# f78bono/deep-cine-cardiac-mri

Hardware: AMD Instinct MI355X
Metric: cine slices/sec, XF-VarNet R=4 15-coil 200x200x15t (higher is better)
Workload: dtype f32; 1 GPU; BASELINE.json configs[1]: XF-VarNet, 6 cascades, 15 coils x 15 frames x 200x200, R=4 Gaussian-density Cartesian mask, sens net 8ch/3 pools, U-Net 16ch/3 pools; 1 slice(s) per step (k-space batch axis), seeded random-init weights, 9 different slices per rank; parallelism=slice-sharded x1, one all-gather for volume assembly

## Files before the change

deep-cine-cardiac-mri_amd/cine_hip/dc.py:

```python
from typing import Optional

import torch

from . import autograd as ag
from . import ops


class Acquisition:
    def __init__(self, ref_kspace: torch.Tensor, mask: torch.Tensor, sens_maps: torch.Tensor, train: bool = False):
        layout = ops.mask_layout(mask, ref_kspace)
        if layout is None:
            raise ValueError(f"mask {tuple(mask.shape)} is in neither layout for k-space {tuple(ref_kspace.shape)}: pass it through ops.as_mask_u8")
        self.kspace, self.mask, self.sens, self.train = ref_kspace, mask, sens_maps, train
        self.row = layout == "row"
        self.fused = ops.general_mask_fused_train(mask, ref_kspace) if train else (self.row or ops.GENERAL_MASK_FUSED)
        self._hyb = self._zf = self._tiled = self._mf = None

    @property
    def tiled(self) -> Optional[torch.Tensor]:
        if self._tiled is None and self.row and not self.train:
            self._tiled = ops.sens_tile_pack(self.sens)
        return self._tiled

    @property
# ... 8 lines not shown
        self._hyb = ops.kspace_to_hybrid(self.kspace)
        return ops.hybrid_reduce(self._hyb, self.sens)

    def zero_filled(self) -> torch.Tensor:
        if self._zf is None:
            hyb, self._hyb = self._hyb, None
            if self.train:
                self._zf = ag.CoilReduceFn.apply(self.kspace, self.sens, self.mask)
            elif self.row:
                self._zf = ops.hybrid_reduce(ops.kspace_to_hybrid(self.kspace, out=hyb, mask=self.mask), self.sens)
            else:
                del hyb
                self._zf = ops.sens_reduce(ops.apply_mask(self.kspace, self.mask), self.sens, destroy_input=True)
        return self._zf

    def soft_dc(self, img: torch.Tensor, lambda_reg: torch.Tensor, magnitude: bool = False) -> torch.Tensor:
        if self.train:
            if self.row or self.fused:
                return ag.ImageDcFn.apply(img, self.sens, self.zero_filled(), self.mask, lambda_reg)
            k = ops.soft_dc_blend(ag.SensExpandFn.apply(img, self.sens, None), self.kspace, self.mask, lambda_reg)
            return ag.SensReduceFn.apply(k.contiguous(), self.sens, None)
        if self.fused:
            return ops.image_dc(img, self.sens, self.zero_filled(), self.mask, lambda_reg, magnitude=magnitude, sens_tiled=self.tiled)
        k = ops.soft_dc_blend(ops.sens_expand_dc(img, self.sens), self.kspace, self.mask, lambda_reg.detach())
        return ops.sens_reduce(k, self.sens, magnitude=magnitude, destroy_input=True)

    def residual_backward(self, x0: torch.Tensor) -> torch.Tensor:
        if self.train:
            if self.row or self.fused:
                return ag.ImageDcFixedFn.apply(x0, self.sens, self.zero_filled(), self.mask, 1.0, 0.0, -1.0)
            return ag.masked_residual_backward(x0, self.sens, self.kspace, self.mask)
        if self.fused:
            return ops.image_dc(x0, self.sens, self.zero_filled(), self.mask, weights=(1.0, 0.0, -1.0), sens_tiled=self.tiled)
        return ops.masked_residual_backward(x0, self.sens, self.kspace, self.mask)

    def forward_masked(self, x0: torch.Tensor) -> torch.Tensor:
        if self.train:
# ... 27 lines not shown
```

deep-cine-cardiac-mri_amd/cine_hip/ops.py:

```python
from typing import NamedTuple, Optional, Sequence

import contextlib
import ctypes
import threading
import numpy as np
import torch

from ._lib import CineHipError, check, lib

IN_EPS = 1e-5
LRELU_SLOPE = 0.2
RELU_ON = True
_act_tls = threading.local()


def lrelu_slope() -> float:
    return getattr(_act_tls, "slope", LRELU_SLOPE)


def relu_on() -> bool:
    return getattr(_act_tls, "relu", RELU_ON)


@contextlib.contextmanager
# ... 1211 lines not shown
    stats = torch.empty((n, 2, 2), device=x.device, dtype=x.dtype) if norm else None
    check(lib().cine_normunet_pack(x.data_ptr(), planes.data_ptr(), _p(stats), n, h, w, int(norm), _stream()),
          "cine_normunet_pack")
    return planes, stats


def normunet_unpack(planes: torch.Tensor, stats: Optional[torch.Tensor], h: int, w: int) -> torch.Tensor:
    planes = _dev(planes, "planes")
    n = planes.shape[0]
    y = torch.empty((n, h, w, 2), device=planes.device, dtype=planes.dtype)
    check(lib().cine_normunet_unpack(planes.data_ptr(), _p(stats), y.data_ptr(), n, h, w, _stream()),
          "cine_normunet_unpack")
    return y


def xfyf_pack(img: torch.Tensor, xf: bool, norm: bool = True):
    _pair(img)
    img = _dev(img, "image")
    b, t, h, w, _ = img.shape
    dev, dt = img.device, img.dtype
    pd = pad16 if norm else (lambda v: v)
    if pd(w) == pd(h):
        joint = torch.empty((b * h + b * w, 2, pd(w), pd(t)), device=dev, dtype=dt)
        pxf, pyf = joint[:b * h], joint[b * h:]
    else:
        pxf = torch.empty((b * h, 2, pd(w), pd(t)), device=dev, dtype=dt)
        pyf = torch.empty((b * w, 2, pd(h), pd(t)), device=dev, dtype=dt)
    sxf = torch.empty((b * h, 2, 2), device=dev, dtype=dt) if norm else None
    syf = torch.empty((b * w, 2, 2), device=dev, dtype=dt) if norm else None
    mean = torch.empty((b, h, w, 2), device=dev, dtype=dt)
    nbytes = lib().cine_xfyf_ws_bytes(b, t, h, w)
    ws = torch.empty(nbytes, device=dev, dtype=torch.uint8)
    check(lib().cine_xfyf_pack(img.data_ptr(), pxf.data_ptr(), pyf.data_ptr(), _p(sxf), _p(syf),
                               mean.data_ptr(), b, t, h, w, int(xf), int(norm), ws.data_ptr(), nbytes, _stream()),
          "cine_xfyf_pack")
    return pxf, pyf, sxf, syf, mean


def xfyf_unpack(pxf, pyf, sxf, syf, mean, b: int, t: int, h: int, w: int, xf: bool) -> torch.Tensor:
    out = torch.empty((b, t, 1, h, w, 2), device=pxf.device, dtype=pxf.dtype)
    check(lib().cine_xfyf_unpack(_dev(pxf, "pxf").data_ptr(), _dev(pyf, "pyf").data_ptr(), _p(sxf),
                                 _p(syf), mean.data_ptr(), out.data_ptr(), b, t, h, w, int(xf), _stream()),
          "cine_xfyf_unpack")
    return out


class _Kind(NamedTuple):
    stem: str
    dims: tuple
    tail: Optional[tuple]
    op: Optional[int]

    @property
    def floats_fn(self) -> str:
        return f"cine_{self.stem}_packed_floats"

    @property
    def pack_fn(self) -> str:
        return f"cine_pack_{self.stem}"
# ... 607 lines not shown
```

deep-cine-cardiac-mri_amd/csrc/fft_kernels.hip:

```cpp
#include <algorithm>
#include <map>
#include <mutex>
#include <utility>
#include "common.h"
#include "fft_core.h"

namespace cine {

__device__ const float2 TW200[200] = {
#include "tw200.inc"
};

constexpr int kLines200 = 32, kThreads200 = 320;
constexpr int kLinesGen = 8, kThreadsGen = 256;
constexpr int kMaxGenericN = 400;
constexpr int kMaxSmoothN = 512;
constexpr int kMaxOut = 4;

enum { POST_NONE = 0, POST_DC = 1, POST_HARD = 2, POST_RESID = 3, POST_W2D = 4,
       POST_LOSS = 5, POST_LOSSG = 6 };
constexpr bool post_plane(int post) { return post == POST_W2D || post == POST_LOSS || post == POST_LOSSG; }
constexpr bool post_kref(int post) { return post == POST_DC || post == POST_RESID || post == POST_LOSS || post == POST_LOSSG; }
enum { PRE_NONE = 0, PRE_SMUL = 1 };
enum { RPOST_NONE = 0, RPOST_REDUCE = 1, RPOST_REDUCE_ABS = 2, RPOST_RSS = 3,
// ... 1149 lines not shown
        ca.H = h; ca.W = w; ca.s_in = (h + 1) / 2; ca.s_out = h / 2; ca.coils = c;
        ca.premask = mask + (i0 / c) * h;
        if (int e = launch_col<POST_NONE, false, true>(ca, ni, true, st)) return e;
    }
    return CINE_OK;
}

extern "C" size_t cine_image_dc_ws_bytes(int b, int t, int c, int h, int w) {
    if (b <= 0 || t <= 0 || c <= 0 || h != 200 || w <= 0 || c <= kDcCS) return 0;
    return (size_t)ceil_div(c, kDcCS) * b * t * h * w * sizeof(cf);
}

static int image_dc_impl(const float* img, const float* sens, const float* zf, const uint8_t* mask,
                         const float* lambda_dev, int lam_beta, float w_sampled, float w_unsampled, float beta,
                         float* out, int b, int t, int c, int h, int w, int magnitude,
                         void* ws, size_t ws_bytes, void* stream, float* pd_part = nullptr, float* pd_wg = nullptr, const float* sens_tiled = nullptr);

extern "C" int cine_image_dc(const float* img, const float* sens, const float* zf, const uint8_t* mask,
                             const float* lambda_dev, float w_sampled, float w_unsampled, float beta,
                             float* out, int b, int t, int c, int h, int w, int magnitude,
                             void* ws, size_t ws_bytes, void* stream) {
    return image_dc_impl(img, sens, zf, mask, lambda_dev, 0, w_sampled, w_unsampled, beta, out, b, t, c, h, w, magnitude, ws, ws_bytes, stream);
}

extern "C" int cine_normal_op(const float* img, const float* sens, const uint8_t* mask, const float* lambda_dev,
                              float* out, int b, int t, int c, int h, int w, void* ws, size_t ws_bytes, void* stream) {
    CINE_REQUIRE(lambda_dev, CINE_EINVAL, "cine_normal_op: null lambda");
    return image_dc_impl(img, sens, img, mask, lambda_dev, 1, 1.f, 0.f, 0.f, out, b, t, c, h, w, 0, ws, ws_bytes, stream);
}
extern "C" size_t cine_sens_tile_floats(int b, int c, int h, int w) {
    return (b <= 0 || c <= 0 || h != 200 || w <= 0) ? 0 : (size_t)b * c * ceil_div(w, kDcCW) * 200 * kDcCW * 2;
// ... 16 lines not shown
    CINE_REQUIRE(sens && tiled, CINE_EINVAL, "cine_sens_tile_pack: null pointer");
    CINE_REQUIRE(b > 0 && c > 0 && h == 200 && w > 0, CINE_EUNSUPPORTED, "cine_sens_tile_pack: h must be 200 (the only engine that reads the tiled maps)");
    hipStream_t st = as_stream(stream);
    ProfScope prof(F_PACK, st);
    const long total = (long)b * c * ceil_div(w, kDcCW) * 200 * kDcCW;
    hipLaunchKernelGGL(sens_tile_pack_kernel, dim3((unsigned)std::min<long>(ceil_div(total, 256L), 4096)), dim3(256), 0, st,
                       reinterpret_cast<const cf*>(sens), reinterpret_cast<cf*>(tiled), w, ceil_div(w, kDcCW), (long)b * c);
    return check_launch("sens_tile_pack_kernel");
}
extern "C" int cine_image_dc_t(const float* img, const float* sens, const float* sens_tiled, const float* zf, const uint8_t* mask,
                               const float* lambda_dev, float w_sampled, float w_unsampled, float beta,
                               float* out, int b, int t, int c, int h, int w, int magnitude,
                               void* ws, size_t ws_bytes, void* stream) {
    return image_dc_impl(img, sens, zf, mask, lambda_dev, 0, w_sampled, w_unsampled, beta, out, b, t, c, h, w, magnitude, ws, ws_bytes, stream,
                         nullptr, nullptr, sens_tiled);
}
extern "C" int cine_normal_op_t(const float* img, const float* sens, const float* sens_tiled, const uint8_t* mask, const float* lambda_dev,
                                float* out, int b, int t, int c, int h, int w, void* ws, size_t ws_bytes, void* stream) {
    CINE_REQUIRE(lambda_dev, CINE_EINVAL, "cine_normal_op_t: null lambda");
    return image_dc_impl(img, sens, img, mask, lambda_dev, 1, 1.f, 0.f, 0.f, out, b, t, c, h, w, 0, ws, ws_bytes, stream, nullptr, nullptr, sens_tiled);
}
extern "C" int cine_normal_op_pd(const float* img, const float* sens, const uint8_t* mask, const float* lambda_dev,
                                 float* out, float* pd_part, int b, int t, int c, int h, int w, void* ws, size_t ws_bytes, void* stream) {
    CINE_REQUIRE(lambda_dev && pd_part, CINE_EINVAL, "cine_normal_op_pd: null pointer");
    CINE_REQUIRE(cine_image_dc_ws_bytes(b, t, c, h, w) > 0, CINE_EUNSUPPORTED, "cine_normal_op_pd: this shape has no partial-sum kernel");
    return image_dc_impl(img, sens, img, mask, lambda_dev, 1, 1.f, 0.f, 0.f, out, b, t, c, h, w, 0, ws, ws_bytes, stream, pd_part);
}

namespace cine {
int launch_cg_update_fused(float* x, float* r, float* p, const cf* partial, int nz, long part_stride, const float* lam, long ncf,
// ... 93 lines not shown
        a.cg_p_out = pk;
        {
            ProfScope prof(F_FFT_COL, st);
            hipLaunchKernelGGL(imgdc200_kernel<true>, dim3((unsigned)nb), dim3(kDcT), (size_t)200 * kDcL * sizeof(cf), st, a);
            if (int e = check_launch("imgdc200_kernel<cg>")) return e;
        }
        if (int e = launch_cg_update2(x, pr, pk, partial, nz, ncf, lambda_dev, ncf, pd_wg, (int)nb, rr[k & 1], rr[(k + 1) & 1], k + 1 == iters, st,
                                      rr_rec ? rr_rec + k : nullptr, pd_rec ? pd_rec + k : nullptr, (rr_rec && k + 1 == iters) ? rr_rec + iters : nullptr)) return e;
    }
    return CINE_OK;
}

static int image_dc_impl(const float* img, const float* sens, const float* zf, const uint8_t* mask,
                         const float* lambda_dev, int lam_beta, float w_sampled, float w_unsampled, float beta,
                         float* out, int b, int t, int c, int h, int w, int magnitude,
                         void* ws, size_t ws_bytes, void* stream, float* pd_part, float* pd_wg, const float* sens_tiled) {
    CINE_REQUIRE(img && sens && mask && (out || pd_wg), CINE_EINVAL, "cine_image_dc: null pointer");
    CINE_REQUIRE(b > 0 && t > 0 && c > 0 && h > 0 && w > 0, CINE_EINVAL, "cine_image_dc: bad sizes");
    CINE_REQUIRE((long)b * t <= 65535, CINE_EUNSUPPORTED, "cine_image_dc: b*t > 65535");
    CINE_REQUIRE(img != out, CINE_EINVAL, "cine_image_dc: out must not alias img (workgroups read neighbouring columns' rows)");
    if (int e = check_n(h, "cine_image_dc(h)")) return e;
    const size_t need = cine_image_dc_ws_bytes(b, t, c, h, w);
    CINE_REQUIRE(need == 0 || (ws && ws_bytes >= need), CINE_EWORKSPACE, "cine_image_dc: workspace %zu < %zu", ws_bytes, need);
    ImgDcArgs a{};
    a.img = reinterpret_cast<const cf*>(img); a.sens = reinterpret_cast<const cf*>(sens);
    a.zf = reinterpret_cast<const cf*>(zf); a.mask = mask; a.lam = lambda_dev; a.lam_beta = lam_beta;
    a.w1 = w_sampled; a.w0 = w_unsampled; a.beta = beta;
    a.out = magnitude ? nullptr : reinterpret_cast<cf*>(out); a.out_abs = magnitude ? out : nullptr;
    a.T = t; a.C = c; a.H = h; a.W = w;
    hipStream_t st = as_stream(stream);
    ProfScope prof(F_FFT_COL, st);
    if (h == 200) {
        const int nz = ceil_div(c, kDcCS);
        CINE_REQUIRE(nz <= 65535, CINE_EUNSUPPORTED, "cine_image_dc: %d coils", c);
        a.partial = reinterpret_cast<cf*>(ws); a.part_stride = (long)b * t * h * w;
        a.BT = b * t; a.ntx = ceil_div(w, kDcCW); a.nz = nz;
        a.sens_t = reinterpret_cast<const cf*>(sens_tiled);
        const long nblk = 8L * ceil_div(a.ntx * nz, 8) * a.BT;
        CINE_REQUIRE(nblk <= 0x7fffffffL, CINE_EUNSUPPORTED, "cine_image_dc: grid too large");
        CINE_REQUIRE(!pd_wg || nz > 1, CINE_EUNSUPPORTED, "cine_image_dc: per-workgroup dot partials need more than one coil group");
        a.pd_wg = pd_wg;
        hipLaunchKernelGGL(imgdc200_kernel<false>, dim3((unsigned)nblk), dim3(kDcT), (size_t)200 * kDcL * sizeof(cf), st, a);
        if (int e = check_launch("imgdc200_kernel")) return e;
        if (nz > 1 && !pd_wg) {
            const long n = a.part_stride;
            a.pd_part = pd_part;
            hipLaunchKernelGGL(imgdc_sum_kernel, dim3(pd_part ? 256u : (unsigned)std::min<long>(ceil_div(n, 256L), 2048)), dim3(256), 0, st, a, nz, n);
        }
    } else {
        const size_t lds = lds_bytes(false, h, kLinesGen);
        if (int e = allow_lds(imgdc_generic_kernel, lds, "imgdc_generic_kernel")) return e;
        hipLaunchKernelGGL(imgdc_generic_kernel, dim3(ceil_div(w, kLinesGen), b * t), dim3(kThreadsGen), lds, st, a);
    }
    return check_launch("imgdc_kernel");
}

extern "C" int cine_hybrid_reduce(const float* hyb, const float* sens, float* out,
                                  int b, int t, int c, int h, int w, int magnitude, void* stream) {
    CINE_REQUIRE(hyb && sens && out, CINE_EINVAL, "cine_hybrid_reduce: null pointer");
// ... 341 lines not shown
```

deep-cine-cardiac-mri_amd/csrc/pack_kernels.hip:

```cpp
#include <algorithm>
#include "common.h"
#include "fft_core.h"

namespace cine {

__device__ __forceinline__ float wave_sum(float v) {
#pragma unroll
    for (int o = 32; o > 0; o >>= 1) v += __shfl_xor(v, o, 64);
    return v;
}
__device__ __forceinline__ float block_sum(float v, float* red) {
    v = wave_sum(v);
    const int wave = threadIdx.x >> 6, nw = (blockDim.x + 63) >> 6;
    __syncthreads();
    if ((threadIdx.x & 63) == 0) red[wave] = v;
    __syncthreads();
    float s = 0.f;
    for (int i = 0; i < nw; ++i) s += red[i];
    return s;
}

struct PackArgs {
    const float* x; float* planes; float* stats;
    int n, I, J, Ip, Jp, pad_i, pad_j;
// ... 114 lines not shown
    if (stats) { const float* st = stats + (long)n * 4; mr = st[0]; sdr = st[1]; mi = st[2]; sdi = st[3]; }
    const float* pr = planes + (long)n * 2 * Ip * Jp;
    const float* pi = pr + (long)Ip * Jp;
    for (int e = blockIdx.x * blockDim.x + threadIdx.x; e < I * J; e += gridDim.x * blockDim.x) {
        const int i = e / J, j = e - i * J;
        const int q = (i + pad_i) * Jp + (j + pad_j);
        float2 v;
        v.x = pr[q] * sdr + mr;
        v.y = pi[q] * sdi + mi;
        reinterpret_cast<float2*>(y)[(long)n * I * J + e] = v;
    }
}

constexpr int kPix = 64;

__device__ __forceinline__ void temporal_table(cf* tw, int T) {
    const double s = 1.0 / sqrt((double)T);
    for (int j = threadIdx.x; j < T; j += blockDim.x) {
        double sn, cs;
        sincospi(2.0 * (double)j / (double)T, &sn, &cs);
        tw[j] = mk((float)(cs * s), (float)(-sn * s));
    }
}

__global__ void temporal_fwd_kernel(const cf* img, cf* X, cf* mean_img, int T, long HW, int xf) {
    extern __shared__ __align__(16) unsigned char smem[];
    cf* buf = reinterpret_cast<cf*>(smem);
    cf* tw = buf + T * kPix;
    const int b = blockIdx.y;
    const long p0 = (long)blockIdx.x * kPix;
    const int np = (int)min((long)kPix, HW - p0);
    if (xf) temporal_table(tw, T);
    for (int e = threadIdx.x; e < T * kPix; e += blockDim.x) {
        const int t = e / kPix, p = e - t * kPix;
        buf[e] = p < np ? img[((long)b * T + t) * HW + p0 + p] : mk(0.f, 0.f);
    }
    __syncthreads();
    if (threadIdx.x < kPix) {
        const int p = threadIdx.x;
        float sx = 0.f, sy = 0.f;
        for (int t = 0; t < T; ++t) { sx += buf[t * kPix + p].x; sy += buf[t * kPix + p].y; }
        const cf m = mk(sx / T, sy / T);
        for (int t = 0; t < T; ++t) buf[t * kPix + p] = csub(buf[t * kPix + p], m);
        if (p < np) mean_img[(long)b * HW + p0 + p] = m;
    }
    __syncthreads();
    const int s_in = (T + 1) / 2, s_out = T / 2;
    for (int e = threadIdx.x; e < np * T; e += blockDim.x) {
        const int p = e / T, i = e - p * T;
        cf r;
// ... 7 lines not shown
                ax += x.x * w.x - x.y * w.y; ay += x.x * w.y + x.y * w.x;
                idx += k; if (idx >= T) idx -= T;
            }
            r = mk(ax, ay);
        } else {
            r = buf[i * kPix + p];
        }
        X[((long)b * HW + p0 + p) * T + i] = r;
    }
}

struct UnpackArgs {
    const float* pxf; const float* pyf; const float* sxf; const float* syf;
    const cf* mean_img; cf* out;
    int T, H, W, Tp, Hp, Wp, pad_t, pad_h, pad_w, xf;
};

__global__ void xfyf_unpack_kernel(UnpackArgs a) {
    extern __shared__ __align__(16) unsigned char smem[];
    cf* buf = reinterpret_cast<cf*>(smem);
    cf* tw = buf + a.T * kPix;
    const int T = a.T, H = a.H, W = a.W;
    const int b = blockIdx.z, h = blockIdx.y;
    const int w0 = blockIdx.x * kPix;
    const int np = min(kPix, W - w0);
    if (a.xf) temporal_table(tw, T);
    const long nxf = (long)b * H + h;
    float xmr = 0.f, xsr = 1.f, xmi = 0.f, xsi = 1.f;
    if (a.sxf) { const float* sx = a.sxf + nxf * 4; xmr = sx[0]; xsr = sx[1]; xmi = sx[2]; xsi = sx[3]; }
    const float* pxr = a.pxf + nxf * 2 * a.Wp * a.Tp;
    const float* pxi = pxr + (long)a.Wp * a.Tp;
    for (int e = threadIdx.x; e < np * T; e += blockDim.x) {
        const int p = e / T, t = e - p * T;
        const int w = w0 + p;
        const int qx = (w + a.pad_w) * a.Tp + t + a.pad_t;
        const float xr = pxr[qx] * xsr + xmr, xi = pxi[qx] * xsi + xmi;
        const long nyf = (long)b * W + w;
        float ymr = 0.f, ysr = 1.f, ymi = 0.f, ysi = 1.f;
        if (a.syf) { const float* sy = a.syf + nyf * 4; ymr = sy[0]; ysr = sy[1]; ymi = sy[2]; ysi = sy[3]; }
        const float* pyr = a.pyf + nyf * 2 * a.Hp * a.Tp;
        const float* pyi = pyr + (long)a.Hp * a.Tp;
// ... 102 lines not shown
extern "C" int cine_normunet_unpack(const float* planes, const float* stats, float* y, int n, int h, int w, void* stream) {
    CINE_REQUIRE(planes && y, CINE_EINVAL, "cine_normunet_unpack: null pointer");
    CINE_REQUIRE(n > 0 && n <= 65535 && h > 0 && w > 0, CINE_EINVAL, "cine_normunet_unpack: bad sizes");
    int hp, ph, wp, pw;
    pad_split(h, hp, ph, stats != nullptr); pad_split(w, wp, pw, stats != nullptr);
    ProfScope prof(F_PACK, as_stream(stream));
    hipLaunchKernelGGL(normunet_unpack_kernel, dim3(grid_for((long)h * w, 256, 64), n), dim3(256), 0, as_stream(stream),
                       planes, stats, y, h, w, hp, wp, ph, pw);
    return check_launch("normunet_unpack_kernel");
}

extern "C" size_t cine_xfyf_ws_bytes(int b, int t, int h, int w) {
    return (size_t)b * t * h * w * 2 * sizeof(float);
}

extern "C" int cine_xfyf_pack(const float* img, float* planes_xf, float* planes_yf, float* stats_xf, float* stats_yf,
                              float* mean_img, int b, int t, int h, int w, int xf, int norm, void* ws, size_t ws_bytes, void* stream) {
    CINE_REQUIRE(img && planes_xf && planes_yf && mean_img && ws && (!norm || (stats_xf && stats_yf)), CINE_EINVAL,
                 "cine_xfyf_pack: null pointer");
    CINE_REQUIRE(b > 0 && b <= 65535 && t > 1 && h > 0 && w > 0, CINE_EINVAL, "cine_xfyf_pack: bad sizes");
    CINE_REQUIRE(t <= 64, CINE_EUNSUPPORTED, "cine_xfyf_pack: %d frames > 64", t);
    CINE_REQUIRE(ws_bytes >= cine_xfyf_ws_bytes(b, t, h, w), CINE_EWORKSPACE, "cine_xfyf_pack: workspace too small");
    hipStream_t st = as_stream(stream);
    cf* X = reinterpret_cast<cf*>(ws);
    const long HW = (long)h * w;
    const size_t lds = ((size_t)t * kPix + t) * sizeof(cf);
    ProfScope prof(F_PACK, st);
    hipLaunchKernelGGL(temporal_fwd_kernel, dim3((unsigned)ceil_div(HW, (long)kPix), b), dim3(256), lds, st,
                       reinterpret_cast<const cf*>(img), X, reinterpret_cast<cf*>(mean_img), t, HW, xf);
    if (int e = check_launch("temporal_fwd_kernel")) return e;
    PackArgs a{};
    a.x = reinterpret_cast<const float*>(X); a.planes = planes_xf; a.stats = stats_xf;
    a.n = b * h; a.I = w; a.J = t; a.norm = norm != 0;
    pad_split(w, a.Ip, a.pad_i, a.norm); pad_split(t, a.Jp, a.pad_j, a.norm);
    a.ninner = h; a.s_outer = HW * t * 2; a.s_inner = (long)w * t * 2; a.si = (long)t * 2; a.sj = 2;
    const PackArgs axf = a;
    a.planes = planes_yf; a.stats = stats_yf;
    a.n = b * w; a.I = h; a.J = t;
    pad_split(h, a.Ip, a.pad_i, a.norm); pad_split(t, a.Jp, a.pad_j, a.norm);
    a.ninner = w; a.s_outer = HW * t * 2; a.s_inner = (long)t * 2; a.si = (long)w * t * 2; a.sj = 2;
    return launch_pack(axf, &a, st);
}

extern "C" int cine_xfyf_unpack(const float* planes_xf, const float* planes_yf, const float* stats_xf,
                                const float* stats_yf, const float* mean_img, float* out,
                                int b, int t, int h, int w, int xf, void* stream) {
    CINE_REQUIRE(planes_xf && planes_yf && mean_img && out && ((stats_xf != nullptr) == (stats_yf != nullptr)), CINE_EINVAL,
                 "cine_xfyf_unpack: null pointer");
    CINE_REQUIRE(b > 0 && t > 1 && t <= 64 && h > 0 && w > 0 && h <= 65535 && b <= 65535, CINE_EINVAL,
                 "cine_xfyf_unpack: bad sizes");
    UnpackArgs a{};
    a.pxf = planes_xf; a.pyf = planes_yf; a.sxf = stats_xf; a.syf = stats_yf;
    a.mean_img = reinterpret_cast<const cf*>(mean_img); a.out = reinterpret_cast<cf*>(out);
    a.T = t; a.H = h; a.W = w; a.xf = xf;
    const bool nrm = stats_xf != nullptr;
    pad_split(t, a.Tp, a.pad_t, nrm); pad_split(h, a.Hp, a.pad_h, nrm); pad_split(w, a.Wp, a.pad_w, nrm);
    const size_t lds = ((size_t)t * kPix + t) * sizeof(cf);
    ProfScope prof(F_PACK, as_stream(stream));
    hipLaunchKernelGGL(xfyf_unpack_kernel, dim3(ceil_div(w, kPix), h, b), dim3(256), lds, as_stream(stream), a);
    return check_launch("xfyf_unpack_kernel");
}

static int sens_prologue_impl(const float* k, float* out, int b, int t, int c, int h, int w, int row_lo, int row_hi, const int* win, void* stream) {
    CINE_REQUIRE(k && out, CINE_EINVAL, "cine_sens_prologue: null pointer");
    CINE_REQUIRE(b > 0 && b <= 65535 && t > 0 && c > 0 && h > 0 && w > 0, CINE_EINVAL, "cine_sens_prologue: bad sizes");
    CINE_REQUIRE(cine_fft_line_supported(h) && cine_fft_line_supported(w), CINE_EUNSUPPORTED, "cine_sens_prologue: FFT size %d x %d unsupported", h, w);
    { ProfScope prof(F_MISC, as_stream(stream));
    hipLaunchKernelGGL(time_mean_center_kernel, dim3(grid_for((long)c * h * w, 256), b), dim3(256), 0, as_stream(stream),
                       reinterpret_cast<const cf*>(k), reinterpret_cast<cf*>(out), t, c, h, w, row_lo, row_hi, win); }
    if (int e = check_launch("time_mean_center_kernel")) return e;
    return cine_fft2c(out, out, b * c, h, w, 1, stream);
}
// ... 410 lines not shown
```

deep-cine-cardiac-mri_amd/reconstruction/models/varnet.py:

```python
import math
from typing import Optional

import torch
from torch import nn

from cine_hip import autograd as ag
from cine_hip import ops
from cine_hip.dc import Acquisition
from .denoisers.norm_unet import NormUnet, NormUnet3D


class SensitivityModel(nn.Module):
    def __init__(self, chans: int, num_pools: int, in_chans: int = 2, out_chans: int = 2, drop_prob: float = 0.0):
        super().__init__()
        self.norm_unet = NormUnet(chans, num_pools, in_chans=in_chans, out_chans=out_chans, drop_prob=drop_prob)

    @staticmethod
    def acs_window(mask: torch.Tensor):
        if mask.shape[-2] != 1:
            raise ValueError("the ACS window is read from a row mask (reference varnet.py:64-68 indexes the mask's h axis); with a mask that "
                             "varies along w pass acs=(pad, n_low) or sens_maps")
        rows = mask[:, 0].reshape(-1).cpu()
        cent = mask.shape[-3] // 2
        left = int(torch.nonzero(rows[:cent] == 0)[-1])
# ... 26 lines not shown

    def sens_expand(self, x: torch.Tensor, sens_maps: torch.Tensor) -> torch.Tensor:
        return ops.sens_expand_dc(x, sens_maps)

    def sens_reduce(self, x: torch.Tensor, sens_maps: torch.Tensor) -> torch.Tensor:
        return ops.sens_reduce(x, sens_maps)

    def _xfyf_weights(self):
        uw = self.model.__dict__.get("_hip_uw")
        if uw is None:
            nets = [self.model, self.model] if self.weight_sharing else [self.model[0], self.model[1]]
            uw = self.model.__dict__["_hip_uw"] = (ops.UnetWeights([nets[0].unet, nets[1].unet]),
                                                    ops.UnetWeights([nets[0].unet]), ops.UnetWeights([nets[1].unet]))
        return uw

    def xfyf_transform(self, image_combined: torch.Tensor) -> torch.Tensor:
        b, t, h, w, _ = image_combined.shape
        xf = self.dynamic_type == 'XF'
        both, wx, wy = self._xfyf_weights()
        if ag.grad_mode(self) or both.drops():
            return ag.xfyf(image_combined, xf, both, wx, wy)
        pxf, pyf, sxf, syf, mean = ops.xfyf_pack(image_combined, xf)
        if pxf.shape == pyf.shape and pxf.data_ptr() + pxf.numel() * 4 == pyf.data_ptr():
            joint = torch.as_strided(pxf, (2 * pxf.shape[0],) + tuple(pxf.shape[1:]), pxf.stride())
            out = ops.unet2d_forward(joint, both)
            oxf, oyf = out[:pxf.shape[0]], out[pxf.shape[0]:]
        else:
            oxf, oyf = ops.unet2d_forward(pxf, wx), ops.unet2d_forward(pyf, wy)
        return ops.xfyf_unpack(oxf, oyf, sxf, syf, mean, b, t, h, w, xf)

    def regularise(self, image_combined: torch.Tensor) -> torch.Tensor:
        if self.dynamic_type in ['XF', 'XT']:
            return self.xfyf_transform(image_combined.squeeze(2))
        if self.dynamic_type == '2D':
            return self.model(image_combined.squeeze(0)).unsqueeze(0)
        if self.dynamic_type == '3D':
            return self.model(image_combined.permute(0, 2, 1, 3, 4, 5)).permute(0, 2, 1, 3, 4, 5).contiguous()
        raise ValueError(f"unknown dynamic_type {self.dynamic_type!r}")

    def forward(self, current_kspace, ref_kspace, mask, sens_maps):
        model_out = self.regularise(ops.sens_reduce(current_kspace, sens_maps))
        if mask.shape[-2] > 1:
            return ops.soft_dc_blend(ops.sens_expand_dc(model_out, sens_maps), ref_kspace, mask, self.lambda_reg.detach())
        return ops.sens_expand_dc(model_out, sens_maps, ref_kspace, mask, self.lambda_reg)


class VarNet(nn.Module):
# ... 21 lines not shown
            return self._forward_infer(masked_kspace, mask, sens_maps, acs, cplx)

    def _forward_train(self, masked_kspace, mask, sens_maps, acs, cplx=False):
        return self._cascade_chain(masked_kspace, mask, sens_maps, acs, True, cplx)

    def _forward_infer(self, masked_kspace, mask, sens_maps, acs, cplx=False):
        return self._cascade_chain(masked_kspace, mask, sens_maps, acs, False, cplx)

    def _cascade_chain(self, masked_kspace, mask, sens_maps, acs, train, cplx=False):
        if sens_maps is None:
            sens_maps = self.sens_net(masked_kspace, mask, acs)
        acq = Acquisition(masked_kspace, mask, sens_maps, train)
        image = acq.image()
        last = None if train or cplx else len(self.cascades) - 1
        for i, cascade in enumerate(self.cascades):
            image = acq.soft_dc(cascade.regularise(image), cascade.lambda_reg, magnitude=(i == last))
        if cplx:
            return image.squeeze(2)
        if train:
            return ag.AbsFn.apply(image.squeeze(2))
        return image if self.cascades else ops.complex_abs(image.squeeze(2))
```

include/cine_hip.h:

```cpp
#ifndef CINE_HIP_H
#define CINE_HIP_H

#include <stddef.h>
#include <stdint.h>

#ifdef __cplusplus
extern "C" {
#endif

#define CINE_OK 0
#define CINE_EINVAL (-1)
#define CINE_EUNSUPPORTED (-2)
#define CINE_EWORKSPACE (-3)
#define CINE_EHIP (-4)

int cine_version(void);
const char* cine_last_error(void);
const char* cine_build_arch(void);


int cine_fft2c(const float* in, float* out, int nimg, int h, int w, int inverse, void* stream);
int cine_fft_line_supported(int n);

int cine_fft1c(const float* in, float* out, long nlines, int n, int inverse, int variant, void* stream);
// ... 65 lines not shown


int cine_pad16(int n);

int cine_normunet_pack(const float* x, float* planes, float* stats, int n, int h, int w, int norm, void* stream);

int cine_normunet_unpack(const float* planes, const float* stats, float* y, int n, int h, int w, void* stream);

size_t cine_xfyf_ws_bytes(int b, int t, int h, int w);
int cine_xfyf_pack(const float* img, float* planes_xf, float* planes_yf, float* stats_xf, float* stats_yf,
                   float* mean_img, int b, int t, int h, int w, int xf, int norm, void* ws, size_t ws_bytes, void* stream);

int cine_xfyf_unpack(const float* planes_xf, const float* planes_yf, const float* stats_xf,
                     const float* stats_yf, const float* mean_img, float* out,
                     int b, int t, int h, int w, int xf, void* stream);


size_t cine_conv3x3_packed_floats(int cout, int cin);
size_t cine_tconv2x2_packed_floats(int cin, int cout);
size_t cine_conv1x1_packed_floats(int cout, int cin);
int cine_pack_conv3x3(const float* w, float* packed, int cout, int cin, void* stream);
int cine_pack_tconv2x2(const float* w, float* packed, int cin, int cout, void* stream);
int cine_pack_conv1x1(const float* w, float* packed, int cout, int cin, void* stream);

int cine_conv_stat_partials(int cout, int h, int w, int is_tconv);

int cine_conv3x3_in(const float* x0, const float* part0, int np0, int c0, int mode0, int h0, int w0,
                    const float* x1, const float* part1, int np1, int c1, int mode1, int h1, int w1,
                    const float* wpacked, const float* wpacked2, int set_split,
                    float* y, float* part_y, int n, int cout, int h, int w, float eps, float slope, void* stream);
// ... 337 lines not shown
```

Before: 174.9 cine slices/sec.

## Fuse coil-group partial-sum reduction of image DC into next cascade's xf/yf pack

```diff
diff --git a/deep-cine-cardiac-mri_amd/cine_hip/dc.py b/deep-cine-cardiac-mri_amd/cine_hip/dc.py
--- a/deep-cine-cardiac-mri_amd/cine_hip/dc.py
+++ b/deep-cine-cardiac-mri_amd/cine_hip/dc.py
@@ -46,13 +46,17 @@
                 self._zf = ops.sens_reduce(ops.apply_mask(self.kspace, self.mask), self.sens, destroy_input=True)
         return self._zf
 
-    def soft_dc(self, img: torch.Tensor, lambda_reg: torch.Tensor, magnitude: bool = False) -> torch.Tensor:
+    def soft_dc(self, img: torch.Tensor, lambda_reg: torch.Tensor, magnitude: bool = False, groups: bool = False):
         if self.train:
             if self.row or self.fused:
                 return ag.ImageDcFn.apply(img, self.sens, self.zero_filled(), self.mask, lambda_reg)
             k = ops.soft_dc_blend(ag.SensExpandFn.apply(img, self.sens, None), self.kspace, self.mask, lambda_reg)
             return ag.SensReduceFn.apply(k.contiguous(), self.sens, None)
         if self.fused:
+            if groups and self.row and not magnitude:
+                sums = ops.image_dc_groups(img, self.sens, self.zero_filled(), self.mask, lambda_reg, sens_tiled=self.tiled)
+                if sums is not None:
+                    return sums
             return ops.image_dc(img, self.sens, self.zero_filled(), self.mask, lambda_reg, magnitude=magnitude, sens_tiled=self.tiled)
         k = ops.soft_dc_blend(ops.sens_expand_dc(img, self.sens), self.kspace, self.mask, lambda_reg.detach())
         return ops.sens_reduce(k, self.sens, magnitude=magnitude, destroy_input=True)
diff --git a/deep-cine-cardiac-mri_amd/cine_hip/ops.py b/deep-cine-cardiac-mri_amd/cine_hip/ops.py
--- a/deep-cine-cardiac-mri_amd/cine_hip/ops.py
+++ b/deep-cine-cardiac-mri_amd/cine_hip/ops.py
@@ -1249,10 +1249,17 @@
     return y
 
 
-def xfyf_pack(img: torch.Tensor, xf: bool, norm: bool = True):
-    _pair(img)
-    img = _dev(img, "image")
-    b, t, h, w, _ = img.shape
+def xfyf_pack(img, xf: bool, norm: bool = True, chain: bool = False):
+    sums = img if isinstance(img, CoilGroupSums) else None
+    if sums is not None:
+        if not (chain and norm):
+            raise ValueError("xfyf_pack: coil-group sums need chain=True and norm=True")
+        b, t, h, w = sums.shape
+        img = sums.partial
+    else:
+        _pair(img)
+        img = _dev(img, "image")
+        b, t, h, w, _ = img.shape
     dev, dt = img.device, img.dtype
     pd = pad16 if norm else (lambda v: v)
     if pd(w) == pd(h):
@@ -1266,18 +1273,61 @@
     mean = torch.empty((b, h, w, 2), device=dev, dtype=dt)
     nbytes = lib().cine_xfyf_ws_bytes(b, t, h, w)
     ws = torch.empty(nbytes, device=dev, dtype=torch.uint8)
+    if chain and norm:
+        head = (img.data_ptr(), None, 0, None, None, 0.0) if sums is None else \
+            (None, sums.partial.data_ptr(), sums.partial.shape[0], _p(sums.zf), sums.lam.data_ptr(), 0.0)
+        check(lib().cine_xfyf_pack_sums(*head, pxf.data_ptr(), pyf.data_ptr(), sxf.data_ptr(), syf.data_ptr(), mean.data_ptr(),
+                                        b, t, h, w, int(xf), ws.data_ptr(), nbytes, _stream()), "cine_xfyf_pack_sums")
+        return pxf, pyf, sxf, syf, mean
     check(lib().cine_xfyf_pack(img.data_ptr(), pxf.data_ptr(), pyf.data_ptr(), _p(sxf), _p(syf),
                                mean.data_ptr(), b, t, h, w, int(xf), int(norm), ws.data_ptr(), nbytes, _stream()),
           "cine_xfyf_pack")
     return pxf, pyf, sxf, syf, mean
 
 
-def xfyf_unpack(pxf, pyf, sxf, syf, mean, b: int, t: int, h: int, w: int, xf: bool) -> torch.Tensor:
+def xfyf_unpack(pxf, pyf, sxf, syf, mean, b: int, t: int, h: int, w: int, xf: bool, table: bool = False) -> torch.Tensor:
     out = torch.empty((b, t, 1, h, w, 2), device=pxf.device, dtype=pxf.dtype)
-    check(lib().cine_xfyf_unpack(_dev(pxf, "pxf").data_ptr(), _dev(pyf, "pyf").data_ptr(), _p(sxf),
-                                 _p(syf), mean.data_ptr(), out.data_ptr(), b, t, h, w, int(xf), _stream()),
+    fn = lib().cine_xfyf_unpack_tab if table else lib().cine_xfyf_unpack
+    check(fn(_dev(pxf, "pxf").data_ptr(), _dev(pyf, "pyf").data_ptr(), _p(sxf),
+             _p(syf), mean.data_ptr(), out.data_ptr(), b, t, h, w, int(xf), _stream()),
           "cine_xfyf_unpack")
     return out
+
+
+CHAIN_UNFUSED_BIT = 32
+
+
+def chain_fused() -> bool:
+    return not (conv_plane_mask() & CHAIN_UNFUSED_BIT)
+
+
+class CoilGroupSums(NamedTuple):
+    partial: torch.Tensor
+    zf: Optional[torch.Tensor]
+    lam: torch.Tensor
+    shape: tuple
+
+
+def image_dc_groups(img: torch.Tensor, sens: torch.Tensor, zf: Optional[torch.Tensor], mask: torch.Tensor, lambda_reg: torch.Tensor,
+                    sens_tiled: Optional[torch.Tensor] = None) -> Optional[CoilGroupSums]:
+    _pair(img); _pair(sens)
+    img = _dev(img, "image"); sens = _dev(sens, "sens_maps"); mask = _dev(mask, "mask", torch.uint8)
+    b, _, c, h, w, _ = sens.shape
+    t = img.shape[1]
+    nz = lib().cine_image_dc_group_count(b, t, c, h, w)
+    if nz == 0:
+        return None
+    if img.numel() != b * t * h * w * 2 or mask.numel() != b * t * h:
+        raise ValueError(f"image_dc_groups: image {tuple(img.shape)} / row mask {tuple(mask.shape)} do not match sens_maps {tuple(sens.shape)}")
+    if zf is not None:
+        zf = _dev(zf, "zero-filled image")
+        if zf.numel() != img.numel():
+            raise ValueError("image_dc_groups: zero-filled image shape mismatch")
+    lam = _dev(lambda_reg.detach(), "lambda_reg")
+    partial = torch.empty((nz, b, t, h, w, 2), device=img.device, dtype=img.dtype)
+    check(lib().cine_image_dc_groups(img.data_ptr(), sens.data_ptr(), _p(sens_tiled), mask.data_ptr(), lam.data_ptr(), 1.0, 0.0,
+                                     b, t, c, h, w, partial.data_ptr(), partial.numel() * 4, _stream()), "cine_image_dc_groups")
+    return CoilGroupSums(partial, zf, lam, (b, t, h, w))
 
 
 class _Kind(NamedTuple):
diff --git a/deep-cine-cardiac-mri_amd/csrc/fft_kernels.hip b/deep-cine-cardiac-mri_amd/csrc/fft_kernels.hip
--- a/deep-cine-cardiac-mri_amd/csrc/fft_kernels.hip
+++ b/deep-cine-cardiac-mri_amd/csrc/fft_kernels.hip
@@ -1187,7 +1187,8 @@
 static int image_dc_impl(const float* img, const float* sens, const float* zf, const uint8_t* mask,
                          const float* lambda_dev, int lam_beta, float w_sampled, float w_unsampled, float beta,
                          float* out, int b, int t, int c, int h, int w, int magnitude,
-                         void* ws, size_t ws_bytes, void* stream, float* pd_part = nullptr, float* pd_wg = nullptr, const float* sens_tiled = nullptr);
+                         void* ws, size_t ws_bytes, void* stream, float* pd_part = nullptr, float* pd_wg = nullptr, const float* sens_tiled = nullptr,
+                         bool groups_only = false);
 
 extern "C" int cine_image_dc(const float* img, const float* sens, const float* zf, const uint8_t* mask,
                              const float* lambda_dev, float w_sampled, float w_unsampled, float beta,
@@ -1234,6 +1235,17 @@
                                void* ws, size_t ws_bytes, void* stream) {
     return image_dc_impl(img, sens, zf, mask, lambda_dev, 0, w_sampled, w_unsampled, beta, out, b, t, c, h, w, magnitude, ws, ws_bytes, stream,
                          nullptr, nullptr, sens_tiled);
+}
+extern "C" int cine_image_dc_group_count(int b, int t, int c, int h, int w) {
+    return cine_image_dc_ws_bytes(b, t, c, h, w) ? ceil_div(c, kDcCS) : 0;
+}
+extern "C" int cine_image_dc_groups(const float* img, const float* sens, const float* sens_tiled, const uint8_t* mask,
+                                    const float* lambda_dev, float w_sampled, float w_unsampled,
+                                    int b, int t, int c, int h, int w, void* groups, size_t groups_bytes, void* stream) {
+    CINE_REQUIRE(cine_image_dc_group_count(b, t, c, h, w) > 0, CINE_EUNSUPPORTED, "cine_image_dc_groups: this shape has no coil groups (h == 200 and more than %d coils)", kDcCS);
+    CINE_REQUIRE(groups, CINE_EINVAL, "cine_image_dc_groups: null pointer");
+    return image_dc_impl(img, sens, nullptr, mask, lambda_dev, 0, w_sampled, w_unsampled, 0.f, nullptr, b, t, c, h, w, 0, groups, groups_bytes, stream,
+                         nullptr, nullptr, sens_tiled, true);
 }
 extern "C" int cine_normal_op_t(const float* img, const float* sens, const float* sens_tiled, const uint8_t* mask, const float* lambda_dev,
                                 float* out, int b, int t, int c, int h, int w, void* ws, size_t ws_bytes, void* stream) {
@@ -1357,8 +1369,8 @@
 static int image_dc_impl(const float* img, const float* sens, const float* zf, const uint8_t* mask,
                          const float* lambda_dev, int lam_beta, float w_sampled, float w_unsampled, float beta,
                          float* out, int b, int t, int c, int h, int w, int magnitude,
-                         void* ws, size_t ws_bytes, void* stream, float* pd_part, float* pd_wg, const float* sens_tiled) {
-    CINE_REQUIRE(img && sens && mask && (out || pd_wg), CINE_EINVAL, "cine_image_dc: null pointer");
+                         void* ws, size_t ws_bytes, void* stream, float* pd_part, float* pd_wg, const float* sens_tiled, bool groups_only) {
+    CINE_REQUIRE(img && sens && mask && (out || pd_wg || groups_only), CINE_EINVAL, "cine_image_dc: null pointer");
     CINE_REQUIRE(b > 0 && t > 0 && c > 0 && h > 0 && w > 0, CINE_EINVAL, "cine_image_dc: bad sizes");
     CINE_REQUIRE((long)b * t <= 65535, CINE_EUNSUPPORTED, "cine_image_dc: b*t > 65535");
     CINE_REQUIRE(img != out, CINE_EINVAL, "cine_image_dc: out must not alias img (workgroups read neighbouring columns' rows)");
@@ -1385,7 +1397,7 @@
         a.pd_wg = pd_wg;
         hipLaunchKernelGGL(imgdc200_kernel<false>, dim3((unsigned)nblk), dim3(kDcT), (size_t)200 * kDcL * sizeof(cf), st, a);
         if (int e = check_launch("imgdc200_kernel")) return e;
-        if (nz > 1 && !pd_wg) {
+        if (nz > 1 && !pd_wg && !groups_only) {
             const long n = a.part_stride;
             a.pd_part = pd_part;
             hipLaunchKernelGGL(imgdc_sum_kernel, dim3(pd_part ? 256u : (unsigned)std::min<long>(ceil_div(n, 256L), 2048)), dim3(256), 0, st, a, nz, n);
diff --git a/deep-cine-cardiac-mri_amd/csrc/pack_kernels.hip b/deep-cine-cardiac-mri_amd/csrc/pack_kernels.hip
--- a/deep-cine-cardiac-mri_amd/csrc/pack_kernels.hip
+++ b/deep-cine-cardiac-mri_amd/csrc/pack_kernels.hip
@@ -1,4 +1,5 @@
 #include <algorithm>
+#include <mutex>
 #include "common.h"
 #include "fft_core.h"
 
@@ -152,26 +153,81 @@
 
 constexpr int kPix = 64;
 
+__device__ __forceinline__ cf temporal_entry(int j, int T) {
+    const double s = 1.0 / sqrt((double)T);
+    double sn, cs;
+    sincospi(2.0 * (double)j / (double)T, &sn, &cs);
+    return mk((float)(cs * s), (float)(-sn * s));
+}
 __device__ __forceinline__ void temporal_table(cf* tw, int T) {
-    const double s = 1.0 / sqrt((double)T);
-    for (int j = threadIdx.x; j < T; j += blockDim.x) {
-        double sn, cs;
-        sincospi(2.0 * (double)j / (double)T, &sn, &cs);
-        tw[j] = mk((float)(cs * s), (float)(-sn * s));
-    }
-}
-
-__global__ void temporal_fwd_kernel(const cf* img, cf* X, cf* mean_img, int T, long HW, int xf) {
+    for (int j = threadIdx.x; j < T; j += blockDim.x) tw[j] = temporal_entry(j, T);
+}
+constexpr int kMaxFrames = 64;
+__device__ cf g_temporal_tab[(kMaxFrames + 1) * kMaxFrames];
+__global__ __launch_bounds__(256) void temporal_tab_fill_kernel() {
+    const int e = blockIdx.x * 256 + threadIdx.x;
+    const int T = e / kMaxFrames, j = e - T * kMaxFrames;
+    if (T >= 2 && T <= kMaxFrames && j < T) g_temporal_tab[e] = temporal_entry(j, T);
+}
+
+struct TemporalSrc {
+    const cf* img;
+    const cf* partial; int nz; long part_stride;
+    const cf* zf; const float* lam; float beta;
+    const cf* ttab;
+};
+
+__global__ void temporal_fwd_kernel(TemporalSrc a, cf* X, cf* mean_img, int T, long HW, int xf) {
     extern __shared__ __align__(16) unsigned char smem[];
     cf* buf = reinterpret_cast<cf*>(smem);
     cf* tw = buf + T * kPix;
     const int b = blockIdx.y;
     const long p0 = (long)blockIdx.x * kPix;
     const int np = (int)min((long)kPix, HW - p0);
-    if (xf) temporal_table(tw, T);
-    for (int e = threadIdx.x; e < T * kPix; e += blockDim.x) {
-        const int t = e / kPix, p = e - t * kPix;
-        buf[e] = p < np ? img[((long)b * T + t) * HW + p0 + p] : mk(0.f, 0.f);
+    if (xf) {
+        if (a.ttab) { for (int j = threadIdx.x; j < T; j += blockDim.x) tw[j] = a.ttab[j]; }
+        else temporal_table(tw, T);
+    }
+    if (a.img) {
+        const cf* img = a.img;
+        for (int e = threadIdx.x; e < T * kPix; e += blockDim.x) {
+            const int t = e / kPix, p = e - t * kPix;
+            buf[e] = p < np ? img[((long)b * T + t) * HW + p0 + p] : mk(0.f, 0.f);
+        }
+    } else {
+        float beta = a.beta;
+        if (a.lam) {
+            const float l = *a.lam;
+            const float v = l > 20.f ? l : log1pf(expf(l));
+            const float w1 = 1.0f / (1.f + v);
+            beta = v * w1;
+        }
+        constexpr int U = 4;
+        const int cnt = T * kPix, nt = blockDim.x;
+        for (int e0 = threadIdx.x; e0 < cnt; e0 += U * nt) {
+            long o[U]; cf v[U];
+#pragma unroll
+            for (int u = 0; u < U; ++u) {
+                const int e = min(e0 + u * nt, cnt - 1);
+                const int t = e / kPix, p = min(e - t * kPix, np - 1);
+                o[u] = ((long)b * T + t) * HW + p0 + p;
+            }
+#pragma unroll
+            for (int u = 0; u < U; ++u) v[u] = a.partial[o[u]];
+            for (int z = 1; z < a.nz; ++z) {
+#pragma unroll
+                for (int u = 0; u < U; ++u) { const cf w = a.partial[z * a.part_stride + o[u]]; v[u].x += w.x; v[u].y += w.y; }
+            }
+            if (a.zf) {
+#pragma unroll
+                for (int u = 0; u < U; ++u) { const cf zz = a.zf[o[u]]; v[u].x = fmaf(beta, zz.x, v[u].x); v[u].y = fmaf(beta, zz.y, v[u].y); }
+            }
+#pragma unroll
+            for (int u = 0; u < U; ++u) {
+                const int e = e0 + u * nt;
+                if (e < cnt) buf[e] = (e % kPix) < np ? v[u] : mk(0.f, 0.f);
+            }
+        }
     }
     __syncthreads();
     if (threadIdx.x < kPix) {
@@ -209,6 +265,7 @@
     const float* pxf; const float* pyf; const float* sxf; const float* syf;
     const cf* mean_img; cf* out;
     int T, H, W, Tp, Hp, Wp, pad_t, pad_h, pad_w, xf;
+    const cf* ttab;
 };
 
 __global__ void xfyf_unpack_kernel(UnpackArgs a) {
@@ -219,7 +276,10 @@
     const int b = blockIdx.z, h = blockIdx.y;
     const int w0 = blockIdx.x * kPix;
     const int np = min(kPix, W - w0);
-    if (a.xf) temporal_table(tw, T);
+    if (a.xf) {
+        if (a.ttab) { for (int j = threadIdx.x; j < T; j += blockDim.x) tw[j] = a.ttab[j]; }
+        else temporal_table(tw, T);
+    }
     const long nxf = (long)b * H + h;
     float xmr = 0.f, xsr = 1.f, xmi = 0.f, xsi = 1.f;
     if (a.sxf) { const float* sx = a.sxf + nxf * 4; xmr = sx[0]; xsr = sx[1]; xmi = sx[2]; xsi = sx[3]; }
@@ -352,9 +412,30 @@
     return (size_t)b * t * h * w * 2 * sizeof(float);
 }
 
+static int temporal_table_dev(int t, hipStream_t st, const cf** tab);
+static int xfyf_pack_impl(TemporalSrc src, bool table, float* planes_xf, float* planes_yf, float* stats_xf, float* stats_yf,
+                          float* mean_img, int b, int t, int h, int w, int xf, int norm, void* ws, size_t ws_bytes, void* stream);
 extern "C" int cine_xfyf_pack(const float* img, float* planes_xf, float* planes_yf, float* stats_xf, float* stats_yf,
                               float* mean_img, int b, int t, int h, int w, int xf, int norm, void* ws, size_t ws_bytes, void* stream) {
-    CINE_REQUIRE(img && planes_xf && planes_yf && mean_img && ws && (!norm || (stats_xf && stats_yf)), CINE_EINVAL,
+    CINE_REQUIRE(img, CINE_EINVAL, "cine_xfyf_pack: null pointer");
+    TemporalSrc src{};
+    src.img = reinterpret_cast<const cf*>(img);
+    return xfyf_pack_impl(src, false, planes_xf, planes_yf, stats_xf, stats_yf, mean_img, b, t, h, w, xf, norm, ws, ws_bytes, stream);
+}
+extern "C" int cine_xfyf_pack_sums(const float* img, const float* partial, int nz, const float* zf, const float* lambda_dev, float beta,
+                                   float* planes_xf, float* planes_yf, float* stats_xf, float* stats_yf, float* mean_img,
+                                   int b, int t, int h, int w, int xf, void* ws, size_t ws_bytes, void* stream) {
+    CINE_REQUIRE((img != nullptr) != (partial != nullptr), CINE_EINVAL, "cine_xfyf_pack_sums: give the image or the coil-group sums, not both");
+    CINE_REQUIRE(img || (nz >= 1 && nz <= 65535), CINE_EINVAL, "cine_xfyf_pack_sums: bad number of coil groups");
+    TemporalSrc src{};
+    src.img = reinterpret_cast<const cf*>(img);
+    src.partial = reinterpret_cast<const cf*>(partial); src.nz = nz; src.part_stride = (long)b * t * h * w;
+    src.zf = reinterpret_cast<const cf*>(zf); src.lam = lambda_dev; src.beta = beta;
+    return xfyf_pack_impl(src, true, planes_xf, planes_yf, stats_xf, stats_yf, mean_img, b, t, h, w, xf, 1, ws, ws_bytes, stream);
+}
+static int xfyf_pack_impl(TemporalSrc src, bool table, float* planes_xf, float* planes_yf, float* stats_xf, float* stats_yf,
+                          float* mean_img, int b, int t, int h, int w, int xf, int norm, void* ws, size_t ws_bytes, void* stream) {
+    CINE_REQUIRE(planes_xf && planes_yf && mean_img && ws && (!norm || (stats_xf && stats_yf)), CINE_EINVAL,
                  "cine_xfyf_pack: null pointer");
     CINE_REQUIRE(b > 0 && b <= 65535 && t > 1 && h > 0 && w > 0, CINE_EINVAL, "cine_xfyf_pack: bad sizes");
     CINE_REQUIRE(t <= 64, CINE_EUNSUPPORTED, "cine_xfyf_pack: %d frames > 64", t);
@@ -363,9 +444,10 @@
     cf* X = reinterpret_cast<cf*>(ws);
     const long HW = (long)h * w;
     const size_t lds = ((size_t)t * kPix + t) * sizeof(cf);
+    if (table && xf) { if (int e = temporal_table_dev(t, st, &src.ttab)) return e; }
     ProfScope prof(F_PACK, st);
     hipLaunchKernelGGL(temporal_fwd_kernel, dim3((unsigned)ceil_div(HW, (long)kPix), b), dim3(256), lds, st,
-                       reinterpret_cast<const cf*>(img), X, reinterpret_cast<cf*>(mean_img), t, HW, xf);
+                       src, X, reinterpret_cast<cf*>(mean_img), t, HW, xf);
     if (int e = check_launch("temporal_fwd_kernel")) return e;
     PackArgs a{};
     a.x = reinterpret_cast<const float*>(X); a.planes = planes_xf; a.stats = stats_xf;
@@ -380,9 +462,43 @@
     return launch_pack(axf, &a, st);
 }
 
+static int temporal_table_dev(int t, hipStream_t st, const cf** tab) {
+    static std::mutex mu;
+    static bool filled[64] = {};
+    int dev = 0;
+    if (hipGetDevice(&dev) != hipSuccess || dev < 0 || dev >= 64) { set_error("temporal table: no current device"); return CINE_EHIP; }
+    void* base = nullptr;
+    if (hipGetSymbolAddress(&base, HIP_SYMBOL(g_temporal_tab)) != hipSuccess || !base) { set_error("temporal table: no symbol"); return CINE_EHIP; }
+    *tab = reinterpret_cast<const cf*>(base) + (long)t * kMaxFrames;
+    std::lock_guard<std::mutex> lock(mu);
+    if (filled[dev]) return CINE_OK;
+    hipStreamCaptureStatus cap = hipStreamCaptureStatusNone;
+    if (hipStreamIsCapturing(st, &cap) != hipSuccess) { (void)hipGetLastError(); cap = hipStreamCaptureStatusNone; }
+    hipLaunchKernelGGL(temporal_tab_fill_kernel, dim3(ceil_div((kMaxFrames + 1) * kMaxFrames, 256)), dim3(256), 0, st);
+    if (int e = check_launch("temporal_tab_fill_kernel")) return e;
+    if (cap == hipStreamCaptureStatusNone) {
+        if (hipStreamSynchronize(st) != hipSuccess) { set_error("temporal table: synchronize failed"); return CINE_EHIP; }
+        filled[dev] = true;
+    }
+    return CINE_OK;
+}
+
+static int xfyf_unpack_impl(const float* planes_xf, const float* planes_yf, const float* stats_xf,
+                            const float* stats_yf, const float* mean_img, float* out,
+                            int b, int t, int h, int w, int xf, int table, void* stream);
 extern "C" int cine_xfyf_unpack(const float* planes_xf, const float* planes_yf, const float* stats_xf,
                                 const float* stats_yf, const float* mean_img, float* out,
                                 int b, int t, int h, int w, int xf, void* stream) {
+    return xfyf_unpack_impl(planes_xf, planes_yf, stats_xf, stats_yf, mean_img, out, b, t, h, w, xf, 0, stream);
+}
+extern "C" int cine_xfyf_unpack_tab(const float* planes_xf, const float* planes_yf, const float* stats_xf,
+                                    const float* stats_yf, const float* mean_img, float* out,
+                                    int b, int t, int h, int w, int xf, void* stream) {
+    return xfyf_unpack_impl(planes_xf, planes_yf, stats_xf, stats_yf, mean_img, out, b, t, h, w, xf, 1, stream);
+}
+static int xfyf_unpack_impl(const float* planes_xf, const float* planes_yf, const float* stats_xf,
+                            const float* stats_yf, const float* mean_img, float* out,
+                            int b, int t, int h, int w, int xf, int table, void* stream) {
     CINE_REQUIRE(planes_xf && planes_yf && mean_img && out && ((stats_xf != nullptr) == (stats_yf != nullptr)), CINE_EINVAL,
                  "cine_xfyf_unpack: null pointer");
     CINE_REQUIRE(b > 0 && t > 1 && t <= 64 && h > 0 && w > 0 && h <= 65535 && b <= 65535, CINE_EINVAL,
@@ -394,6 +510,7 @@
     const bool nrm = stats_xf != nullptr;
     pad_split(t, a.Tp, a.pad_t, nrm); pad_split(h, a.Hp, a.pad_h, nrm); pad_split(w, a.Wp, a.pad_w, nrm);
     const size_t lds = ((size_t)t * kPix + t) * sizeof(cf);
+    if (table && xf) { if (int e = temporal_table_dev(t, as_stream(stream), &a.ttab)) return e; }
     ProfScope prof(F_PACK, as_stream(stream));
     hipLaunchKernelGGL(xfyf_unpack_kernel, dim3(ceil_div(w, kPix), h, b), dim3(256), lds, as_stream(stream), a);
     return check_launch("xfyf_unpack_kernel");
diff --git a/deep-cine-cardiac-mri_amd/reconstruction/models/varnet.py b/deep-cine-cardiac-mri_amd/reconstruction/models/varnet.py
--- a/deep-cine-cardiac-mri_amd/reconstruction/models/varnet.py
+++ b/deep-cine-cardiac-mri_amd/reconstruction/models/varnet.py
@@ -64,23 +64,33 @@
                                                     ops.UnetWeights([nets[0].unet]), ops.UnetWeights([nets[1].unet]))
         return uw
 
-    def xfyf_transform(self, image_combined: torch.Tensor) -> torch.Tensor:
-        b, t, h, w, _ = image_combined.shape
+    def takes_group_sums(self) -> bool:
+        return (self.dynamic_type in ['XF', 'XT'] and ops.chain_fused()
+                and not ag.grad_mode(self) and not self._xfyf_weights()[0].drops())
+
+    def xfyf_transform(self, image_combined) -> torch.Tensor:
+        sums = isinstance(image_combined, ops.CoilGroupSums)
+        b, t, h, w = image_combined.shape if sums else image_combined.shape[:4]
         xf = self.dynamic_type == 'XF'
         both, wx, wy = self._xfyf_weights()
         if ag.grad_mode(self) or both.drops():
             return ag.xfyf(image_combined, xf, both, wx, wy)
-        pxf, pyf, sxf, syf, mean = ops.xfyf_pack(image_combined, xf)
+        fused = ops.chain_fused()
+        if sums and not fused:
+            raise ValueError("coil-group sums need the chain form of the front half: ask takes_group_sums() first")
+        pxf, pyf, sxf, syf, mean = ops.xfyf_pack(image_combined, xf, chain=fused)
         if pxf.shape == pyf.shape and pxf.data_ptr() + pxf.numel() * 4 == pyf.data_ptr():
             joint = torch.as_strided(pxf, (2 * pxf.shape[0],) + tuple(pxf.shape[1:]), pxf.stride())
             out = ops.unet2d_forward(joint, both)
             oxf, oyf = out[:pxf.shape[0]], out[pxf.shape[0]:]
         else:
             oxf, oyf = ops.unet2d_forward(pxf, wx), ops.unet2d_forward(pyf, wy)
-        return ops.xfyf_unpack(oxf, oyf, sxf, syf, mean, b, t, h, w, xf)
+        return ops.xfyf_unpack(oxf, oyf, sxf, syf, mean, b, t, h, w, xf, table=fused)
 
-    def regularise(self, image_combined: torch.Tensor) -> torch.Tensor:
+    def regularise(self, image_combined) -> torch.Tensor:
         if self.dynamic_type in ['XF', 'XT']:
+            if isinstance(image_combined, ops.CoilGroupSums):
+                return self.xfyf_transform(image_combined)
             return self.xfyf_transform(image_combined.squeeze(2))
         if self.dynamic_type == '2D':
             return self.model(image_combined.squeeze(0)).unsqueeze(0)
@@ -132,7 +142,9 @@
         image = acq.image()
         last = None if train or cplx else len(self.cascades) - 1
         for i, cascade in enumerate(self.cascades):
-            image = acq.soft_dc(cascade.regularise(image), cascade.lambda_reg, magnitude=(i == last))
+            nxt = self.cascades[i + 1] if i + 1 < len(self.cascades) else None
+            groups = not train and nxt is not None and nxt.takes_group_sums()
+            image = acq.soft_dc(cascade.regularise(image), cascade.lambda_reg, magnitude=(i == last), groups=groups)
         if cplx:
             return image.squeeze(2)
         if train:
diff --git a/include/cine_hip.h b/include/cine_hip.h
--- a/include/cine_hip.h
+++ b/include/cine_hip.h
@@ -103,6 +103,17 @@
 int cine_xfyf_unpack(const float* planes_xf, const float* planes_yf, const float* stats_xf,
                      const float* stats_yf, const float* mean_img, float* out,
                      int b, int t, int h, int w, int xf, void* stream);
+
+int cine_xfyf_unpack_tab(const float* planes_xf, const float* planes_yf, const float* stats_xf,
+                         const float* stats_yf, const float* mean_img, float* out,
+                         int b, int t, int h, int w, int xf, void* stream);
+int cine_image_dc_group_count(int b, int t, int c, int h, int w);
+int cine_image_dc_groups(const float* img, const float* sens, const float* sens_tiled, const uint8_t* mask,
+                         const float* lambda_dev, float w_sampled, float w_unsampled,
+                         int b, int t, int c, int h, int w, void* groups, size_t groups_bytes, void* stream);
+int cine_xfyf_pack_sums(const float* img, const float* partial, int nz, const float* zf, const float* lambda_dev, float beta,
+                        float* planes_xf, float* planes_yf, float* stats_xf, float* stats_yf, float* mean_img,
+                        int b, int t, int h, int w, int xf, void* ws, size_t ws_bytes, void* stream);
 
 
 size_t cine_conv3x3_packed_floats(int cout, int cin);
```

Result: no change. 175.4 cine slices/sec, median of 6 (+0.3%).
